# aghasemzadeh/OpenMPL

Measured on AMD Instinct MI355X. Metric: poses/sec (V=4, J=17, batch=1024 per GPU) fp32, higher is better.
Workload: dtype f32; 1 GPU; Human3.6M config: V=4 J=17 batch=1024 fp32, CHOSEN flag set, depth 12, DIM 32, heads 8; global_batch=1024, parallelism=single GPU

## Files before the change

openmpl_amd/csrc/h2_phase.hpp:

```cpp
#pragma once
#include <mutex>
#include <type_traits>

#include "gemm_common.hpp"

namespace mpl {

typedef _Float16 f16x8 __attribute__((ext_vector_type(8)));
typedef __bf16 bf16x8 __attribute__((ext_vector_type(8)));
typedef unsigned u32x4 __attribute__((ext_vector_type(4)));
typedef unsigned u32x2 __attribute__((ext_vector_type(2)));

constexpr int H2_RG = 2 * 1024;
constexpr int H2_A = 4 * H2_RG;
constexpr int H2_W = 18 * 1024;
constexpr int H2_STAGE = H2_A + H2_W;
constexpr int H2_NST = 6;
constexpr int H2_VEC = H2_NST * H2_STAGE;
constexpr int H2_LDS_BYTES = H2_VEC + 4096;
constexpr int H2_DW_RES = 80 * 1024;
constexpr int H2_FAIL = H2_VEC + 4092;
constexpr int H2_T0 = 5;
constexpr int H2_MAX_WGS = 1024;
constexpr int H2_ATT_TS = 3 * BN + 4;
// ... 173 lines not shown
        const float4 a = pv4(row, 32 * p + 4 * kq), b = pv4(row, 32 * p + 16 + 4 * kq);
        float4 sa = {1.f, 1.f, 1.f, 1.f}, sb = {1.f, 1.f, 1.f, 1.f};
        if (NP == 2) { sa = ld4(so + 32 * p + 4 * kq); sb = ld4(so + 32 * p + 16 + 4 * kq); }
        const float x[8] = {a.x * sa.x, a.y * sa.y, a.z * sa.z, a.w * sa.w, b.x * sb.x, b.y * sb.y, b.z * sb.z, b.w * sb.w};
        h2_emit_frag<NP>(WT, cbase, 4 * g_out + p, (unsigned)(rg * strip + (kq * 16 + li) * 16), x);
    }
    for (int t = tid; t < BM * 2; t += 512) {
        const int li = t & 15, kq = (t >> 4) & 1, rg = t >> 5;
        if (rg < rg_lo || rg >= rg_lo + rgs) continue;
        const int row = rg * 16 + li;
        const float4 a = pv4(row, 128 + 4 * kq);
        float4 sa = {1.f, 1.f, 1.f, 1.f};
        if (NP == 2) sa = ld4(so + 128 + 4 * kq);
        const float x[8] = {a.x * sa.x, a.y * sa.y, a.z * sa.z, a.w * sa.w, 0.f, 0.f, 0.f, 0.f};
        h2_emit_tail<NP>(WT, cbase, 4 * Go + (g_out >> 2), (unsigned)(rg * strip + ((g_out & 3) * 16 + li) * 16 + kq * 8), x,
                         ((Dq / BK) & 1) && (g_out >> 2) == (Go >> 2) - 1);
    }
}

__device__ __forceinline__ bool h2_att_in_registers(int ntok, int hd, int rpt) {
    return (ntok == 2 || ntok == 4 || ntok == 8) && (hd == 68 || hd == BN) && rpt == BM;
}

template <int EPI, bool LNF, int NPASS, int NTW, bool CHAIN, int WC, int RT = 1, int NP = 2, bool ACT = true, bool DW = false>
__device__ __forceinline__ bool h2_phase(const H2Args& a, char* smem, int tid, int wave, int slot0, int tm, int tn,
                                         unsigned* chain, unsigned chain_need, bool arrive = true, int rg_lo = 0, int rgs = 4) {
    static_assert(ACT || (RT == 1 && CHAIN), "loader-only waves exist in the row-narrow stack only");
    static_assert(!DW || (RT == 1 && CHAIN && NP == 2), "direct-W form: 16-row teams of the fp16x2 stack");
    constexpr int ABYTES = RT * 4 * H2_RG;
    constexpr int STAGE = ABYTES + H2_W;
    constexpr int NST = RT == 1 ? H2_NST : 4;
    constexpr int APW = 2 * RT;
    static_assert(NST * STAGE <= H2_VEC, "ring too large");
    static_assert(RT == 1 || (RT == 2 && CHAIN && NP == 2 && EPI != H2_EPI_ATT && NPASS <= 2), "two row tiles per stage: proj / fc1 / fc2 of the fp16x2 stack");
    constexpr bool RAWX = LNF && NP == 2;
    constexpr bool P2 = RT == 1;
    constexpr int DIST = P2 ? NST - 1 : NST;
    constexpr bool LEAD = NTW == H2_T0;
    constexpr bool HAS_A = LEAD && ACT;
    const bool WT = CHAIN && !a.plain;
    const int lane = tid & 63;
    const int rg = DW ? rg_lo : (wave & 3);
    const int li = lane & 15, kq = lane >> 4;
    const int M = a.M, N = a.N, K = a.K;
    const int m0 = tm * RT * a.rpt, n0 = NPASS == 2 ? tn * (2 * BN) : tn * BN;
    const int Dq = N / 3;
    const int KT = h2_ksteps(K, NP), G = K / BN;
    const int T = NPASS * KT;
    auto colbase = [&](int pass) -> int { return NPASS == 3 ? pass * Dq + n0 : n0 + pass * BN; };
    const unsigned long long t_entry = (H2_DBG && a.dbg) ? __builtin_amdgcn_s_memtime() : 0;

    const int row_l = rg * 16 + li;
    bool row_ok[RT];
    int row[RT];
#pragma unroll
    for (int rt = 0; rt < RT; ++rt) {
        row_ok[rt] = row_l < a.rpt && m0 + rt * a.rpt + row_l < M;
        row[rt] = row_ok[rt] ? m0 + rt * a.rpt + row_l : (M - 1);
    }

    const int w_first = RT == 1 ? (LEAD ? 10 + 2 * wave : (wave < 6 ? 3 * (wave - 4) : 6 + 2 * (wave - 6)))
                                : (LEAD ? 14 + wave : (wave < 6 ? 4 * (wave - 4) : 8 + 3 * (wave - 6)));
    static_assert(RT == 1 ? (LEAD ? WC == H2_WC0 : (WC == H2_WC1 || WC == H2_WC2))
                          : (LEAD ? WC == H2_R2_WC0 : (WC == H2_R2_WC1 || WC == H2_R2_WC2)), "W pieces per wave");
    constexpr int w_cnt = WC;
    unsigned voW = (unsigned)(lane * 16 + w_first * 1024);
    unsigned voA[RT], voT[RT];
#pragma unroll
    for (int rt = 0; rt < RT; ++rt) {
        voA[rt] = (unsigned)(lane * 16);
        voT[rt] = 0;
        if (RAWX) {
            voA[rt] = (unsigned)(((size_t)(row[rt] - m0) * a.ldx + 4 * kq) * 4);
            voT[rt] = (unsigned)(((size_t)(row[rt] - m0) * a.ldx + 136 * kq + 128) * 4);
        }
        asm volatile("" : "+v"(voA[rt]), "+v"(voT[rt]));
    }
    asm volatile("" : "+v"(voW));
    const unsigned lds0 = (unsigned)(uintptr_t)(__attribute__((address_space(3))) char*)smem;
    int iw_t = 0, iw_g = 0, ia_t = 0, ia_kt = 0;
    unsigned iw_slot = 0, ia_slot = 0;
    const char* is_w[NPASS];
#pragma unroll
    for (int g = 0; g < NPASS; ++g) is_w[g] = a.W2 + (size_t)(colbase(g) / BN) * KT * H2_W;
    const char* is_a[RT];
#pragma unroll
    for (int rt = 0; rt < RT; ++rt)
        is_a[rt] = RAWX ? reinterpret_cast<const char*>(a.X + (size_t)m0 * a.ldx)
                       : a.A2 + (((size_t)tm * RT + rt) * 4 + (wave & 3)) * KT * H2_RG;
    int hotc[NPASS];
#pragma unroll
    for (int g = 0; g < NPASS; ++g) {
        hotc[g] = 0;
        if (H2_ABL & 64) is_w[g] = a.W2 + (size_t)tn * 17 * H2_W;
    }
    auto adv_w = [&](int g) {
        is_w[g] += H2_W;
        if (H2_ABL & 64) {
            if (++hotc[g] == (NP == 2 ? 16 : 8)) {
                hotc[g] = 0;
                is_w[g] -= (NP == 2 ? 16 : 8) * H2_W;
            }
        }
    };
// ... 22 lines not shown
                    asm volatile("s_mov_b32 m0, %2\n\ts_nop 0\n\tglobal_load_lds_dwordx4 %0, %1\n\tglobal_load_lds_dwordx4 %0, %1 offset:1024"
                                 : : "v"(voA[rt]), "s"(is_a[rt]), "s"(dst) : "memory");
                is_a[rt] += H2_RG;
            } else {
                const bool full = ia_kt < 4 * G;
                const char* src = full ? is_a[rt] + (size_t)(136 * (ia_kt >> 2) + 32 * (ia_kt & 3)) * 4 : is_a[rt] + (size_t)(136 * 4 * (ia_kt - 4 * G)) * 4;
                const char* src2 = src + (full ? 64 : 16);
                const unsigned vo = full ? voA[rt] : voT[rt];
                if (CHAIN)
                    asm volatile("s_mov_b32 m0, %3\n\ts_nop 0\n\tglobal_load_lds_dwordx4 %0, %1 sc1\n\ts_mov_b32 m0, %4\n\ts_nop 0\n\tglobal_load_lds_dwordx4 %0, %2 sc1"
                                 : : "v"(vo), "s"(src), "s"(src2), "s"(dst), "s"(dst + 1024u) : "memory");
                else
                    asm volatile("s_mov_b32 m0, %3\n\ts_nop 0\n\tglobal_load_lds_dwordx4 %0, %1\n\ts_mov_b32 m0, %4\n\ts_nop 0\n\tglobal_load_lds_dwordx4 %0, %2"
                                 : : "v"(vo), "s"(src), "s"(src2), "s"(dst), "s"(dst + 1024u) : "memory");
            }
        }
        ++ia_kt;
    };
    auto issue_w = [&]() {
        const unsigned keep = dma_m0_save();
#pragma unroll
        for (int g = 0; g < NPASS; ++g)
            if (g == iw_g) {
                w_pieces(is_w[g], lds0 + iw_slot + (unsigned)(ABYTES + w_first * 1024));
                adv_w(g);
            }
        if (++iw_g == NPASS) iw_g = 0;
        dma_m0_restore(keep);
        ++iw_t;
        iw_slot += STAGE;
        if (iw_slot == NST * STAGE) iw_slot = 0;
    };
    auto issue_a = [&]() {
        if ((ia_t % NPASS) == 0 && HAS_A) {
            const unsigned keep = dma_m0_save();
            a_pieces(ia_slot);
            dma_m0_restore(keep);
        }
        ++ia_t;
        ia_slot += STAGE;
        if (ia_slot == NST * STAGE) ia_slot = 0;
    };
    auto refill_fast = [&](auto wp_c, auto ai_c, unsigned slot) {
        constexpr int g = decltype(wp_c)::value;
        constexpr bool with_a = decltype(ai_c)::value;
        const unsigned keep = dma_m0_save();
        w_pieces(is_w[g], lds0 + slot + (unsigned)(ABYTES + w_first * 1024));
// ... 53 lines not shown
        dw_fetch(std::integral_constant<int, 1>{}, 1 / NPASS);
        dw_fetch(std::integral_constant<int, 2>{}, 2 / NPASS);
        if constexpr (PD == 4) dw_fetch(std::integral_constant<int, 3>{}, 3 / NPASS);
    } else {
        issue_w();
    }
    if (CHAIN) {
        if (!LEAD && wave == 7 && !arrived) {
            const unsigned lim = 1u << a.spin_log2;
            unsigned spin = 0;
            for (; spin < lim; ++spin) {
                if (__hip_atomic_load(chain, __ATOMIC_RELAXED, __HIP_MEMORY_SCOPE_AGENT) >= chain_need) break;
                __builtin_amdgcn_s_sleep(2);
            }
            if (spin == lim && lane == 0) {
                *reinterpret_cast<volatile unsigned*>(smem + H2_FAIL) = 1u;
                if (a.err_ws) __hip_atomic_store(a.err_ws, 1u, __ATOMIC_RELAXED, __HIP_MEMORY_SCOPE_AGENT);
                if (a.err_host) __hip_atomic_store(a.err_host, 1u, __ATOMIC_RELAXED, __HIP_MEMORY_SCOPE_SYSTEM);
                asm volatile("s_waitcnt vmcnt(0) lgkmcnt(0)" ::: "memory");
            }
        }
        __builtin_amdgcn_s_barrier();
        asm volatile("" ::: "memory");
        if (*reinterpret_cast<volatile unsigned*>(smem + H2_FAIL)) {
            asm volatile("s_waitcnt vmcnt(0)" ::: "memory");
            return false;
        }
    }
    const unsigned long long t_chain = (H2_DBG == 2 && a.dbg) ? __builtin_amdgcn_s_memtime() : 0;
    if constexpr (!DW) {
        issue_a();
    } else {
        const int rows_lo = m0 + rg_lo * 16 + li;
        const int rowa = (rg_lo * 16 + li < a.rpt && rows_lo < M) ? rows_lo : (M - 1);
        const unsigned vA = RAWX ? (unsigned)(((size_t)(rowa - m0) * a.ldx + 4 * kq) * 4) : (unsigned)(lane * 16);
        const unsigned vT = RAWX ? (unsigned)(((size_t)(rowa - m0) * a.ldx + 136 * kq + 128) * 4) : 0u;
        const char* abase = RAWX ? reinterpret_cast<const char*>(a.X + (size_t)m0 * a.ldx) : a.A2 + ((size_t)tm * 4 + rg_lo) * KT * H2_RG;
        const unsigned keep = dma_m0_save();
        for (int i = wave; i < 2 * KT; i += 8) {
            const int kt = i >> 1, half = i & 1;
            const char* src;
            unsigned vo;
            if (RAWX) {
                const bool full = kt < 4 * G;
                src = full ? abase + (size_t)(136 * (kt >> 2) + 32 * (kt & 3)) * 4 + half * 64 : abase + (size_t)(136 * 4 * (kt - 4 * G)) * 4 + half * 16;
                vo = full ? vA : vT;
            } else {
                src = abase + (size_t)i * 1024;
                vo = vA;
            }
            asm volatile("s_mov_b32 m0, %2\n\ts_nop 0\n\tglobal_load_lds_dwordx4 %0, %1 sc1" : : "v"(vo), "s"(src), "s"(lds0 + (unsigned)i * 1024u) : "memory");
        }
        dma_m0_restore(keep);
    }
    constexpr unsigned ST_LDS = DW ? 72u * 1024u  : (RT == 2 ? NST * STAGE : STAGE);
    constexpr bool ST_DMA = NPASS >= 2 || RT == 2;
    static_assert(RT == 1 || ST_LDS + 16384 <= H2_VEC, "statistics rows overlap the epilogue vectors");
    float4 st_raw[4];
    if (LNF) {
        const int ns = K / BN;
        if constexpr (ST_DMA) {
            const int hpr = ns >> 1;
            if (lane < 16 * hpr) {
                const unsigned inv = 65536u / (unsigned)hpr + 1u;
                const int lq = (int)(((unsigned)lane * inv) >> 16);
#pragma unroll
                for (int rt = 0; rt < RT; ++rt) {
                    int r = m0 + rt * a.rpt + 16 * rg + lq;
                    r = r < M ? r : M - 1;
                    const float* g = a.stats + ((size_t)r * ns + 2 * (lane - lq * hpr)) * 2;
                    unsigned keep;
                    if (CHAIN)
                        asm volatile("s_mov_b32 %0, m0\n\ts_mov_b32 m0, %2\n\ts_nop 0\n\tglobal_load_lds_dwordx4 %1, off sc1\n\ts_mov_b32 m0, %0"
                                     : "=&s"(keep) : "v"(g), "s"(lds0 + ST_LDS + (unsigned)(wave * 1024 + rt * 8192)) : "memory");
                    else
                        asm volatile("s_mov_b32 %0, m0\n\ts_mov_b32 m0, %2\n\ts_nop 0\n\tglobal_load_lds_dwordx4 %1, off\n\ts_mov_b32 m0, %0"
                                     : "=&s"(keep) : "v"(g), "s"(lds0 + ST_LDS + (unsigned)(wave * 1024 + rt * 8192)) : "memory");
                }
            }
        } else {

            const float* sp = a.stats + (size_t)row[0] * ns * 2;
#pragma unroll
            for (int i = 0; i < 4; ++i) st_raw[i] = (2 * i < ns) ? ld4(sp + 4 * i) : float4{0.f, 0.f, 0.f, 0.f};
        }
    }
    if constexpr (!DW) {
#pragma unroll
        for (int t = 1; t < DIST; ++t) {
            issue_w();
            issue_a();
        }
    }
    const float ainv = (!LNF && a.a_inv) ? a.a_inv[0] : 1.0f;

    float4 rv[RT][NTW];
    auto epilogue_operands = [&]() {
        if constexpr (EPI == H2_EPI_RES && DW) {
#pragma unroll
            for (int n = 0; n < NTW; ++n)
// ... 60 lines not shown
        const f16x8* bs = reinterpret_cast<const f16x8*>(smem + slot + ABYTES) + slot0 * 2 * 64 + lane;
#pragma unroll
        for (int n = 0; n < NTW; ++n) {
            f[n][0] = bs[(n * 2 + 0) * 64];
            f[n][1] = bs[(n * 2 + 1) * 64];
        }
    };
    auto slot_after = [&](unsigned sl) -> unsigned { return sl + STAGE == NST * STAGE ? 0u : sl + STAGE; };
    auto mfma_row = [&](f32x4 (&accp)[RT][NTW], const f16x8 (&af)[RT][2], int ap, const f16x8 (&bf)[NTW][2], int bp) {
#pragma unroll
        for (int rt = 0; rt < RT; ++rt)
#pragma unroll
            for (int n = 0; n < NTW; ++n)
                if (!(H2_ABL & 8)) {
                    if constexpr (NP == 2)
                        accp[rt][n] = __builtin_amdgcn_mfma_f32_16x16x32_f16(bf[n][bp], af[rt][ap], accp[rt][n], 0, 0, 0);
                    else
                        accp[rt][n] = __builtin_amdgcn_mfma_f32_16x16x32_bf16(__builtin_bit_cast(bf16x8, bf[n][bp]), __builtin_bit_cast(bf16x8, af[rt][ap]),
                                                                              accp[rt][n], 0, 0, 0);
                }
    };
    unsigned long long t_land = 0;
    {
        if constexpr (DW) {
            asm volatile("s_waitcnt vmcnt(0)" ::: "memory");
        } else if (HAS_A) {
            constexpr int LATER = P2 ? 2 * WC + APW * (NPASS == 1 ? 2 : 1) : (DIST - 1) * WC + APW * ((DIST - 1) / NPASS);
            static_assert(LATER < 64, "vmcnt is 6 bits");
            asm volatile("s_waitcnt vmcnt(%0)" ::"n"(LATER) : "memory");
        } else {
            asm volatile("s_waitcnt vmcnt(%0)" ::"n"(P2 ? 2 * WC : (DIST - 1) * WC) : "memory");
        }
        if (H2_DBG == 2 && a.dbg) t_land = __builtin_amdgcn_s_memtime();
        {
            if (LNF) {
                const int ns = K / BN;
#pragma unroll
                for (int rt = 0; rt < RT; ++rt) {
                    if constexpr (ST_DMA) {
                        const float* sl = reinterpret_cast<const float*>(smem + ST_LDS + wave * 1024 + rt * 8192) + li * ns * 2;
#pragma unroll
                        for (int i = 0; i < 4; ++i) st_raw[i] = (2 * i < ns) ? ld4(sl + 4 * i) : float4{0.f, 0.f, 0.f, 0.f};
                    }
                    float st[16];
#pragma unroll
                    for (int i = 0; i < 4; ++i) {
                        st[4 * i] = st_raw[i].x; st[4 * i + 1] = st_raw[i].y; st[4 * i + 2] = st_raw[i].z; st[4 * i + 3] = st_raw[i].w;
                    }
                    float msum = 0.f;
#pragma unroll
                    for (int i = 0; i < 8; ++i) msum += (i < ns) ? st[2 * i] : 0.f;
                    const float mean = msum / (float)ns;
                    float m2 = 0.f;
#pragma unroll
                    for (int i = 0; i < 8; ++i) {
                        const float d = st[2 * i] - mean;
                        m2 += (i < ns) ? fmaf((float)BN * d, d, st[2 * i + 1]) : 0.f;
                    }
                    const float rs = 1.0f / sqrtf(fmaf(m2, 1.0f / (float)K, a.eps));
                    if constexpr (NP == 2) {
                        cv_a[rt] = row_ok[rt] ? rs * H2_SA : 0.f;
                        cv_b[rt] = row_ok[rt] ? -mean * (rs * H2_SA) : 0.f;
                    } else {
                        cv_a[rt] = rs;
                        cv_b[rt] = mean;
                    }
                }
                asm volatile("s_waitcnt lgkmcnt(0)" ::: "memory");
            }
        }
        __builtin_amdgcn_s_barrier();
        asm volatile("" ::: "memory");
        if constexpr (ACT && !DW) {
            read_a(0, A0);
            if (RAWX) finish_a(A0);
            read_b(0, B0);
        }
        if constexpr (DW && RAWX) {
            for (int kt = wave; kt < KT; kt += 8) {
                char* p = smem + kt * 2048 + lane * 16;
                cvr0[0] = *reinterpret_cast<const float4*>(p);
                cvr1[0] = *reinterpret_cast<const float4*>(p + 1024);
                finish_a(A0);
                *reinterpret_cast<f16x8*>(p) = A0[0][0];
                *reinterpret_cast<f16x8*>(p + 1024) = A0[0][1];
            }
            asm volatile("s_waitcnt lgkmcnt(0)" ::: "memory");
            __builtin_amdgcn_s_barrier();
            asm volatile("" ::: "memory");
        }
    }
    const unsigned long long t_loop = (H2_DBG && a.dbg) ? __builtin_amdgcn_s_memtime() : 0;
    unsigned long long t_vm = 0, t_bar = 0, t_mm = 0;
    unsigned slot_c = 0;
    auto stage = [&](auto rem_c, auto wp_c, f32x4 (&accp)[RT][NTW], const f16x8 (&a_cur)[RT][2], f16x8 (&a_nxt)[RT][2],
                     const f16x8 (&b_cur)[NTW][2], f16x8 (&b_nxt)[NTW][2], auto nha_c, auto sync_c) {
        constexpr int REM = decltype(rem_c)::value;
        constexpr bool FAST = REM == 0;
        constexpr bool SYNC = !(P2 && FAST) || decltype(sync_c)::value;
        constexpr bool next_has_a = decltype(nha_c)::value;
        constexpr bool more = FAST || REM > 1;
        constexpr bool RF = FAST || REM > DIST;
        constexpr int g0 = decltype(wp_c)::value;
        asm volatile("" : "+s"(slot_c));
        const unsigned slot_n = slot_after(slot_c);
        const unsigned slot_p = slot_c == 0 ? (unsigned)((NST - 1) * STAGE) : slot_c - STAGE;
        unsigned long long w0 = 0, w1 = 0;
        if (H2_DBG && a.dbg) w0 = __builtin_amdgcn_s_memtime();
        if (more && SYNC) {
            if (FAST) {
                if (P2) {
                    constexpr int na = ((g0 + 3) % NPASS == 0 ? 1 : 0) + ((g0 + 4) % NPASS == 0 ? 1 : 0);
                    if (HAS_A) asm volatile("s_waitcnt vmcnt(%0)" ::"n"(2 * WC + APW * na) : "memory");
                    else asm volatile("s_waitcnt vmcnt(%0)" ::"n"(2 * WC) : "memory");
                } else {
                    constexpr int na = ((g0 + 2) % NPASS == 0 ? 1 : 0) + ((g0 + 3) % NPASS == 0 ? 1 : 0) +
                                       (NST > 4 ? ((g0 + 4) % NPASS == 0 ? 1 : 0) + ((g0 + 5) % NPASS == 0 ? 1 : 0) : 0);
                    static_assert(NST == 4 || NST == 6, "in-flight stages of the one-barrier-per-stage form");
                    static_assert((NST - 2) * WC + APW * na < 64, "vmcnt is 6 bits");
                    if (HAS_A) asm volatile("s_waitcnt vmcnt(%0)" ::"n"((NST - 2) * WC + APW * na) : "memory");
                    else asm volatile("s_waitcnt vmcnt(%0)" ::"n"((NST - 2) * WC) : "memory");
                }
            } else {
                constexpr int ahead = (REM - 1 < DIST - 1 ? REM - 1 : DIST - 1) - 1;
                constexpr int per = HAS_A ? WC + (NPASS == 1 ? APW : 0) : WC;
                constexpr int allow = ahead > 0 ? ahead * per : 0;
                static_assert(allow < 64, "vmcnt is 6 bits");
                asm volatile("s_waitcnt vmcnt(%0)" ::"n"(allow) : "memory");
            }
            if (H2_DBG && a.dbg) { w1 = __builtin_amdgcn_s_memtime(); t_vm += w1 - w0; }
            asm volatile("s_waitcnt lgkmcnt(0)" ::: "memory");
            if (!(H2_ABL & 32)) __builtin_amdgcn_s_barrier();
            asm volatile("" ::: "memory");
            if (H2_DBG && a.dbg) t_bar += __builtin_amdgcn_s_memtime() - w1;
        }
        const f16x8* bs = reinterpret_cast<const f16x8*>(smem + slot_n + ABYTES) + slot0 * 2 * 64 + lane;
        auto rd_b = [&](int n) {
            if (more && n < NTW && !(H2_ABL & 1)) {
                b_nxt[n][0] = bs[(n * 2 + 0) * 64];
                b_nxt[n][1] = bs[(n * 2 + 1) * 64];
            }
        };
        auto loads = [&]() {
            if constexpr (ACT) {
                if (more && next_has_a && !(H2_ABL & 4)) read_a(slot_n, a_nxt);
                rd_b(0); rd_b(1); rd_b(2); rd_b(3); rd_b(4);
            }
            constexpr int gr = (g0 + DIST) % NPASS;
            if (RF && !(H2_ABL & 2))
                refill_fast(std::integral_constant<int, gr>{}, std::integral_constant<bool, gr == 0>{}, P2 ? slot_p : slot_c);
            if (REM == 4 && ACT) epilogue_operands();
        };
        __builtin_amdgcn_sched_barrier(0);
        if (!LEAD) {
            loads();
            __builtin_amdgcn_sched_barrier(0);
        }
        unsigned long long m0 = 0;
        if (H2_DBG && a.dbg) m0 = __builtin_amdgcn_s_memtime();
        if constexpr (!ACT) {
        } else if constexpr (NP == 2) {
            mfma_row(accp, a_cur, 1, b_cur, 0);
            mfma_row(accp, a_cur, 0, b_cur, 1);
            mfma_row(accp, a_cur, 0, b_cur, 0);
        } else {
            mfma_row(accp, a_cur, 0, b_cur, 0);
            mfma_row(accp, a_cur, 1, b_cur, 1);
        }
        __builtin_amdgcn_sched_barrier(0);
        if (H2_DBG && a.dbg) t_mm += __builtin_amdgcn_s_memtime() - m0;
        if (LEAD) loads();
        if (RAWX && ACT && more && next_has_a && !(H2_ABL & 16)) finish_a(a_nxt);
        __builtin_amdgcn_sched_barrier(0);
// ... 102 lines not shown
            if constexpr (PD == 4 && (PD + 3) % NPASS == 0) {
                if (rest == PD + 3) {
                    do tail(tail, std::integral_constant<int, PD + 3>{}, Z{}); while (--tail_rep);
                }
            }
            epilogue_operands();
        }
    } else {
    int t = 0;
    for (; t + U - 1 + NST < T; t += U) {
        step(R0{}, std::integral_constant<int, 0>{});
        step(R0{}, std::integral_constant<int, 1 % U>{});
        if constexpr (NPASS >= 2) {
            step(R0{}, std::integral_constant<int, 2 % U>{});
            step(R0{}, std::integral_constant<int, 3 % U>{});
        }
        if constexpr (NPASS == 3) {
            step(R0{}, std::integral_constant<int, 4 % U>{});
            step(R0{}, std::integral_constant<int, 5 % U>{});
        }
    }
    constexpr int TAIL_A = (NST + U - 1) / U * U;
    constexpr int TAIL_B = (NST - NPASS + U - 1) / U * U + NPASS;
    if (T - t == TAIL_A) tail(tail, std::integral_constant<int, TAIL_A>{}, std::integral_constant<int, 0>{});
    else tail(tail, std::integral_constant<int, TAIL_B>{}, std::integral_constant<int, 0>{});
    }

    const unsigned long long t_epi = (H2_DBG && a.dbg) ? __builtin_amdgcn_s_memtime() : 0;
    auto tile_of = [&](int n) -> int { return h2_slot_tile(slot0 + n); };
    auto value4 = [&](int p, int rt, int n, float (&v)[4]) {
        const int cl = 16 * tile_of(n) + 4 * kq;
        const bool ok = cl + 3 < BN;
        const float* vecs = reinterpret_cast<const float*>(smem + H2_VEC) + p * 2 * BN + (ok ? cl : 0);
        const float4 cv = ld4(vecs), sv = ld4(vecs + BN);
        const float c4[4] = {cv.x, cv.y, cv.z, cv.w};
        const float s4[4] = {sv.x, sv.y, sv.z, sv.w};
#pragma unroll
        for (int r = 0; r < 4; ++r) {
            float t;
            if constexpr (NP == 2) t = fmaf(acc[p][rt][n][r], LNF ? s4[r] : s4[r] * ainv, c4[r]);
            else if constexpr (LNF) t = fmaf(cv_a[rt], fmaf(-cv_b[rt], s4[r], acc[p][rt][n][r]), c4[r]);
            else t = acc[p][rt][n][r] + c4[r];
            if (EPI == H2_EPI_GELU) t = gelu_as(t);
            v[r] = ok ? t : 0.f;
        }
    };
// ... 65 lines not shown
            for (int n = 0; n < NTW; ++n) {
                const bool h1 = two_heads && 4 * tile_of(n) + kq >= 17;
                float km[4] = {0.f, 0.f, 0.f, 0.f};
                if constexpr (NTK > 4) {
#pragma unroll
                    for (int c = 0; c < 4; ++c) km[c] = mirror(kv[n][c]);
                }
#pragma unroll
                for (int r = 0; r < NTK; ++r) {
                    float d = qv[n][0] * xpart(kv[n][0], km[0], r);
                    d = fmaf(qv[n][1], xpart(kv[n][1], km[1], r), d);
                    d = fmaf(qv[n][2], xpart(kv[n][2], km[2], r), d);
                    d = fmaf(qv[n][3], xpart(kv[n][3], km[3], r), d);
                    s0[r] += h1 ? 0.f : d;
                    s1[r] += h1 ? d : 0.f;
                }
            }
#pragma unroll
            for (int r = 0; r < NTK; ++r) {
                s0[r] = xor16_add(s0[r]); s0[r] = xor32_add(s0[r]);
                s1[r] = xor16_add(s1[r]); s1[r] = xor32_add(s1[r]);
            }
            float* xs = reinterpret_cast<float*>(smem) + rt * (2 * BM * 2 * NTK);
            const int half = slot0 ? 1 : 0;
            __syncthreads();
            if (kq == 0) {
#pragma unroll
                for (int r = 0; r < NTK; ++r) {
                    xs[(half * BM + row_l) * 2 * NTK + r] = s0[r];
                    xs[(half * BM + row_l) * 2 * NTK + NTK + r] = s1[r];
                }
            }
            __syncthreads();
            float p0[NTK], p1[NTK];
            {
                const float scale = 1.0f / sqrtf((float)a.att_hd);
                float t0[NTK], t1[NTK];
#pragma unroll
                for (int r = 0; r < NTK; ++r) {
                    t0[r] = (xs[row_l * 2 * NTK + r] + xs[(BM + row_l) * 2 * NTK + r]) * scale;
                    t1[r] = (xs[row_l * 2 * NTK + NTK + r] + xs[(BM + row_l) * 2 * NTK + NTK + r]) * scale;
                }
                auto softmax = [](const float (&t)[NTK], float (&pr)[NTK]) {
                    float mx = t[0];
#pragma unroll
                    for (int r = 1; r < NTK; ++r) mx = fmaxf(mx, t[r]);
// ... 38 lines not shown
                return __builtin_bit_cast(float, r);
            };
            const bool two_heads = a.att_hd == 68;
            float s0[4] = {0.f, 0.f, 0.f, 0.f}, s1[4] = {0.f, 0.f, 0.f, 0.f};
    #pragma unroll
            for (int n = 0; n < NTW; ++n) {
                const bool h1 = two_heads && 4 * tile_of(n) + kq >= 17;
    #pragma unroll
                for (int j = 0; j < 4; ++j) {
                    float d = qv[n][0] * quad(kv[n][0], j);
                    d = fmaf(qv[n][1], quad(kv[n][1], j), d);
                    d = fmaf(qv[n][2], quad(kv[n][2], j), d);
                    d = fmaf(qv[n][3], quad(kv[n][3], j), d);
                    s0[j] += h1 ? 0.f : d;
                    s1[j] += h1 ? d : 0.f;
                }
            }
    #pragma unroll
            for (int j = 0; j < 4; ++j) {
                s0[j] = xor16_add(s0[j]); s0[j] = xor32_add(s0[j]);
                s1[j] = xor16_add(s1[j]); s1[j] = xor32_add(s1[j]);
            }
            float* xs = reinterpret_cast<float*>(smem) + rt * (2 * BM * 8);
            const int half = slot0 ? 1 : 0;
            __syncthreads();
            if (kq == 0) {
                st4(xs + (half * BM + row_l) * 8, float4{s0[0], s0[1], s0[2], s0[3]});
                st4(xs + (half * BM + row_l) * 8 + 4, float4{s1[0], s1[1], s1[2], s1[3]});
            }
            __syncthreads();
            float p0[4], p1[4];
            {
                const float4 a0 = ld4(xs + row_l * 8), a1 = ld4(xs + row_l * 8 + 4);
                const float4 b0 = ld4(xs + (BM + row_l) * 8), b1 = ld4(xs + (BM + row_l) * 8 + 4);
                const float scale = 1.0f / sqrtf((float)a.att_hd);
                const float t0[4] = {(a0.x + b0.x) * scale, (a0.y + b0.y) * scale, (a0.z + b0.z) * scale, (a0.w + b0.w) * scale};
                const float t1[4] = {(a1.x + b1.x) * scale, (a1.y + b1.y) * scale, (a1.z + b1.z) * scale, (a1.w + b1.w) * scale};
                auto softmax4 = [](const float (&t)[4], float (&pr)[4]) {
                    const float mx = fmaxf(fmaxf(t[0], t[1]), fmaxf(t[2], t[3]));
                    const float e0 = __expf(t[0] - mx), e1 = __expf(t[1] - mx), e2 = __expf(t[2] - mx), e3 = __expf(t[3] - mx);
                    const float inv = 1.0f / ((e0 + e1) + (e2 + e3));
                    pr[0] = e0 * inv; pr[1] = e1 * inv; pr[2] = e2 * inv; pr[3] = e3 * inv;
                };
                softmax4(t0, p0);
                softmax4(t1, p1);
            }
// ... 88 lines not shown
                            for (int r = 0; r < 4; ++r) vals[rt][n][r] *= so4[r];
                        }
                    }
#pragma unroll
                    for (int q = 0; q < 2; ++q) {
                        const float x[8] = {vals[rt][2 * q][0], vals[rt][2 * q][1], vals[rt][2 * q][2], vals[rt][2 * q][3],
                                            vals[rt][2 * q + 1][0], vals[rt][2 * q + 1][1], vals[rt][2 * q + 1][2], vals[rt][2 * q + 1][3]};
                        h2_emit_frag<NP>(WT, cbase, 4 * g_out + (slot0 ? 2 : 0) + q, (unsigned)(lane * 16), x);
                    }
                    if (NTW == H2_T0 && kq < 2) {
                        const float x[8] = {vals[rt][NTW - 1][0], vals[rt][NTW - 1][1], vals[rt][NTW - 1][2], vals[rt][NTW - 1][3], 0.f, 0.f, 0.f, 0.f};
                        h2_emit_tail<NP>(WT, cbase, 4 * Go + (g_out >> 2), (unsigned)(((g_out & 3) * 16 + li) * 16 + kq * 8), x,
                                         ((N / BK) & 1) && (g_out >> 2) == (Go >> 2) - 1);
                    }
                  }
                }
            }
        }
        if (H2_DBG && a.dbg) t_st = __builtin_amdgcn_s_memtime();
        if constexpr (EPI == H2_EPI_RES) {
            if (a.stats_out) {
                constexpr int XR = RT * 64;
                float* xch = reinterpret_cast<float*>(smem);
                const int half = slot0 ? 1 : 0;
                float sum[RT];
#pragma unroll
                for (int rt = 0; rt < RT; ++rt) {
                    sum[rt] = 0.f;
#pragma unroll
                    for (int n = 0; n < NTW; ++n) sum[rt] += (vals[rt][n][0] + vals[rt][n][1]) + (vals[rt][n][2] + vals[rt][n][3]);
                    sum[rt] = xor16_add(sum[rt]);
                    sum[rt] = xor32_add(sum[rt]);
                }
                __syncthreads();
#pragma unroll
                for (int rt = 0; rt < RT; ++rt)
                    if (kq == 0) xch[half * XR + rt * 64 + row_l] = sum[rt];
                __syncthreads();
                float mean[RT];
#pragma unroll
                for (int rt = 0; rt < RT; ++rt) {
                    mean[rt] = (xch[rt * 64 + row_l] + xch[XR + rt * 64 + row_l]) * (1.0f / (float)BN);
                    float q = 0.f;
#pragma unroll
                    for (int n = 0; n < NTW; ++n) {
                        const bool ok = 16 * tile_of(n) + 4 * kq + 3 < BN;
// ... 13 lines not shown
                    if (half == 0 && kq == 0 && row_ok[rt]) {
                        const u32x2 h = {__builtin_bit_cast(unsigned, mean[rt]),
                                         __builtin_bit_cast(unsigned, xch[2 * XR + rt * 64 + row_l] + xch[3 * XR + rt * 64 + row_l])};
                        h2_st8(WT, a.stats_out + (size_t)m0 * Go * 2, (unsigned)(((row[rt] - m0) * Go + n0 / BN) * 8), h);
                    }
            }
        }
    }
    }
    if (CHAIN) {
        asm volatile("s_waitcnt vmcnt(0)" ::: "memory");
        __syncthreads();
        if (tid == 0 && arrive) __hip_atomic_fetch_add(chain, 1u, __ATOMIC_RELAXED, __HIP_MEMORY_SCOPE_AGENT);
    }
    if (H2_DBG && a.dbg) {
        if (!t_st) t_st = __builtin_amdgcn_s_memtime();
        asm volatile("s_waitcnt vmcnt(0)" ::: "memory");
        const unsigned long long t_end = __builtin_amdgcn_s_memtime();
        if (lane == 0) {
            unsigned long long* o = a.dbg + (size_t)(blockIdx.x * 8 + wave) * 8;
            o[0] = t_entry; o[1] = t_loop; o[2] = t_epi; o[3] = t_st; o[4] = t_end; o[5] = t_vm; o[6] = t_bar; o[7] = t_mm;
            if (H2_DBG == 2) { o[5] = t_chain; o[6] = t_land; }
        }
    }
    return true;
}

template <int EPI, bool LNF, int NPASS, int NP = 2>
__global__ __launch_bounds__(512, 2) void h2_gemm_kernel(const H2Args a) {
    extern __shared__ __attribute__((aligned(1024))) char smem[];
    const int tid = threadIdx.x;
    const int wave = __builtin_amdgcn_readfirstlane(tid >> 6);
    int tm, tn;
    {
        const int b = blockIdx.x;
        if ((a.grid_m & 7) == 0) {
            const int per = a.grid_m >> 3;
            const int xcd = b & 7, i = b >> 3;
            tm = xcd * per + (i % per);
            tn = i / per;
        } else {
            tm = b % a.grid_m;
            tn = b / a.grid_m;
        }
    }
    if (wave < 4) h2_phase<EPI, LNF, NPASS, H2_T0, false, H2_WC0, 1, NP>(a, smem, tid, wave, 0, tm, tn, nullptr, 0u);
// ... 39 lines not shown
                  s.spin_log2, plain};
}
template <int NP>
__device__ __forceinline__ H2Args h2_args_res(const H2StackArgs& s, const char* w, bool fc2, int D, int G, int plain) {
    if (H2_ABL & 64) w = s.w[0][0];
    const int K = fc2 ? 2 * D : D;
    const float* v = h2_trailer<NP>(w, D, K);
    return H2Args{fc2 ? s.hid2 : s.att2, nullptr, 0, w, v, v + D, nullptr, nullptr, nullptr, s.x, D, s.x, D, NP == 1 ? s.x16 : nullptr,
                  s.stats, s.M, D, K, s.rpt, s.n_tiles, G, s.eps, 0, 0, s.dbg, s.err_ws, s.err_host, s.spin_log2, plain};
}

__device__ __forceinline__ void h2_publish_xcd(const H2StackArgs& s, int team, int tid) {
    if (tid == 0) {
        unsigned xcc;
        asm volatile("s_getreg_b32 %0, hwreg(HW_REG_XCC_ID)" : "=s"(xcc));
        __hip_atomic_fetch_or(s.xcc + team, 1u << (xcc & 15u), __ATOMIC_RELAXED, __HIP_MEMORY_SCOPE_AGENT);
    }
}
__device__ __forceinline__ int h2_team_on_one_xcd(const H2StackArgs& s, int team) {
    const unsigned m = __hip_atomic_load(s.xcc + team, __ATOMIC_RELAXED, __HIP_MEMORY_SCOPE_AGENT);
    return (s.plain_ok && m != 0u && (m & (m - 1u)) == 0u) ? 1 : 0;
}

template <int NP>
__global__ __launch_bounds__(512, 2) void h2_stack_kernel(const H2StackArgs s) {
    extern __shared__ __attribute__((aligned(1024))) char smem[];
    const int tid = threadIdx.x;
    const int wave_s = __builtin_amdgcn_readfirstlane(tid >> 6);
    const int G = s.G, D = s.D;
    int team, tn;
    {
        const int b = blockIdx.x;
        team = (b & 7) + 8 * ((b >> 3) / G);
        tn = (b >> 3) % G;
        if (team >= s.n_teams) return;
    }
    if (tid == 0) *reinterpret_cast<volatile unsigned*>(smem + H2_FAIL) = 0u;
    h2_publish_xcd(s, team, tid);
    int plain = 0, seen = 0;
    __syncthreads();
    for (int tile0 = team; tile0 < s.n_tiles; tile0 += s.n_teams) {
        unsigned need = 0;
        for (int ph = 0; ph < s.n_phases; ++ph, need += G) {
            if (!seen && ph >= 2) {
                plain = __builtin_amdgcn_readfirstlane(h2_team_on_one_xcd(s, team));
                seen = 1;
            }
            int wvp = wave_s, tile = tile0, tnp = tn;
            asm volatile("" : "+s"(wvp), "+s"(tile), "+s"(tnp));
            int tidp = wvp * 64 + (int)__builtin_amdgcn_mbcnt_hi(~0u, __builtin_amdgcn_mbcnt_lo(~0u, 0u));
            asm volatile("" : "+v"(tidp));
            const int wv = wvp;
            unsigned* ctr = s.counters + tile;
            const char* const* w = s.w[ph >> 2];
            bool ok = true;
            if (s.inject > 0 && ph == s.inject && tile == 0 && tnp == 0) return;
            switch (ph & 3) {
                case 0: {
                    H2Args a = h2_args_qkv<NP>(s, w[0], D, G, plain);
                    if (wv < 4) ok = h2_phase<H2_EPI_ATT, true, 3, H2_T0, true, H2_WC0, 1, NP>(a, smem, tidp, wv, 0, tile, tnp, ctr, need);
                    else if (wv < 6) ok = h2_phase<H2_EPI_ATT, true, 3, NT - H2_T0, true, H2_WC1, 1, NP>(a, smem, tidp, wv, H2_T0, tile, tnp, ctr, need);
                    else ok = h2_phase<H2_EPI_ATT, true, 3, NT - H2_T0, true, H2_WC2, 1, NP>(a, smem, tidp, wv, H2_T0, tile, tnp, ctr, need);
                    break;
                }
                case 2: {
                    H2Args a = h2_args_fc1<NP>(s, w[2], D, G, plain);
                    if (wv < 4) ok = h2_phase<H2_EPI_GELU, true, 2, H2_T0, true, H2_WC0, 1, NP>(a, smem, tidp, wv, 0, tile, tnp, ctr, need);
                    else if (wv < 6) ok = h2_phase<H2_EPI_GELU, true, 2, NT - H2_T0, true, H2_WC1, 1, NP>(a, smem, tidp, wv, H2_T0, tile, tnp, ctr, need);
                    else ok = h2_phase<H2_EPI_GELU, true, 2, NT - H2_T0, true, H2_WC2, 1, NP>(a, smem, tidp, wv, H2_T0, tile, tnp, ctr, need);
                    break;
                }
                default: {
                    const bool fc2 = (ph & 3) == 3;
                    H2Args a = h2_args_res<NP>(s, fc2 ? w[3] : w[1], fc2, D, G, plain);
                    if (wv < 4) ok = h2_phase<H2_EPI_RES, false, 1, H2_T0, true, H2_WC0, 1, NP>(a, smem, tidp, wv, 0, tile, tnp, ctr, need);
                    else if (wv < 6) ok = h2_phase<H2_EPI_RES, false, 1, NT - H2_T0, true, H2_WC1, 1, NP>(a, smem, tidp, wv, H2_T0, tile, tnp, ctr, need);
                    else ok = h2_phase<H2_EPI_RES, false, 1, NT - H2_T0, true, H2_WC2, 1, NP>(a, smem, tidp, wv, H2_T0, tile, tnp, ctr, need);
                    break;
                }
            }
            if (!ok) return;
        }
    }
}

template <int NP>
__global__ __launch_bounds__(512, 2) void h2_stack2_kernel(const H2StackArgs s) {
    static_assert(NP == 2, "the two-tile stage exists in the fp16x2 engine only");
    extern __shared__ __attribute__((aligned(1024))) char smem[];
    const int tid = threadIdx.x;
    const int wave_s = __builtin_amdgcn_readfirstlane(tid >> 6);
    const int G = s.G, D = s.D;
    int team, tn;
    {
        const int b = blockIdx.x;
        team = (b & 7) + 8 * ((b >> 3) / G);
        tn = (b >> 3) % G;
        if (team >= s.n_teams) return;
    }
    if (tid == 0) *reinterpret_cast<volatile unsigned*>(smem + H2_FAIL) = 0u;
// ... 324 lines not shown
```

Baseline: 816,200 poses/s.

## Prefetch next phase's weight tiles into the LDS ring during the current phase tail

Adds a cross-phase weight prefetch to the persistent stack kernel. During the last DIST stages of each GEMM phase, freed ring slots are filled with the next phase's W pieces, and the next phase starts from the ring position left behind and skips reissuing those loads. The aim is to hide the weight-load latency at the start of each phase behind the previous phase's tail and epilogue. The cost is more intricate vmcnt accounting, relocated statistics and exchange buffers, and a risk of LDS overlap between in-flight prefetch and epilogue scratch.

```diff
diff --git a/openmpl_amd/csrc/h2_phase.hpp b/openmpl_amd/csrc/h2_phase.hpp
--- a/openmpl_amd/csrc/h2_phase.hpp
+++ b/openmpl_amd/csrc/h2_phase.hpp
@@ -219,11 +219,22 @@
     return (ntok == 2 || ntok == 4 || ntok == 8) && (hd == 68 || hd == BN) && rpt == BM;
 }
 
-template <int EPI, bool LNF, int NPASS, int NTW, bool CHAIN, int WC, int RT = 1, int NP = 2, bool ACT = true, bool DW = false>
+struct H2Pf {
+    unsigned base;
+    int pre;
+    const char* nw;
+    unsigned pstride;
+    int npass;
+};
+constexpr int H2_PF_MIN_T = 12;
+
+template <int EPI, bool LNF, int NPASS, int NTW, bool CHAIN, int WC, int RT = 1, int NP = 2, bool ACT = true, bool DW = false, bool PF = false>
 __device__ __forceinline__ bool h2_phase(const H2Args& a, char* smem, int tid, int wave, int slot0, int tm, int tn,
-                                         unsigned* chain, unsigned chain_need, bool arrive = true, int rg_lo = 0, int rgs = 4) {
+                                         unsigned* chain, unsigned chain_need, bool arrive = true, int rg_lo = 0, int rgs = 4,
+                                         H2Pf* pf = nullptr) {
     static_assert(ACT || (RT == 1 && CHAIN), "loader-only waves exist in the row-narrow stack only");
     static_assert(!DW || (RT == 1 && CHAIN && NP == 2), "direct-W form: 16-row teams of the fp16x2 stack");
+    static_assert(!PF || (RT == 1 && CHAIN && ACT && !DW), "cross-phase W prefetch: the whole-tile chain form only");
     constexpr int ABYTES = RT * 4 * H2_RG;
     constexpr int STAGE = ABYTES + H2_W;
     constexpr int NST = RT == 1 ? H2_NST : 4;
@@ -245,6 +256,20 @@
     const int KT = h2_ksteps(K, NP), G = K / BN;
     const int T = NPASS * KT;
     auto colbase = [&](int pass) -> int { return NPASS == 3 ? pass * Dq + n0 : n0 + pass * BN; };
+    unsigned ring0 = 0;
+    bool pre = false, pf_on = false;
+    const char* pf_nw = nullptr;
+    unsigned pf_ps = 0;
+    int pf_np = 1;
+    if constexpr (PF) {
+        ring0 = pf->base;
+        pre = pf->pre != 0;
+        pf_nw = pf->nw;
+        pf_ps = pf->pstride;
+        pf_np = pf->npass;
+        pf_on = pf_nw != nullptr && !(H2_ABL & 64);
+        if (EPI == H2_EPI_ATT && !h2_att_in_registers(a.att_ntok, a.att_hd, a.rpt)) pf_on = false;
+    }
     const unsigned long long t_entry = (H2_DBG && a.dbg) ? __builtin_amdgcn_s_memtime() : 0;
 
     const int row_l = rg * 16 + li;
@@ -276,7 +301,7 @@
     asm volatile("" : "+v"(voW));
     const unsigned lds0 = (unsigned)(uintptr_t)(__attribute__((address_space(3))) char*)smem;
     int iw_t = 0, iw_g = 0, ia_t = 0, ia_kt = 0;
-    unsigned iw_slot = 0, ia_slot = 0;
+    unsigned iw_slot = ring0, ia_slot = ring0;
     const char* is_w[NPASS];
 #pragma unroll
     for (int g = 0; g < NPASS; ++g) is_w[g] = a.W2 + (size_t)(colbase(g) / BN) * KT * H2_W;
@@ -345,7 +370,7 @@
 #pragma unroll
         for (int g = 0; g < NPASS; ++g)
             if (g == iw_g) {
-                w_pieces(is_w[g], lds0 + iw_slot + (unsigned)(ABYTES + w_first * 1024));
+                if (!pre) w_pieces(is_w[g], lds0 + iw_slot + (unsigned)(ABYTES + w_first * 1024));
                 adv_w(g);
             }
         if (++iw_g == NPASS) iw_g = 0;
@@ -445,7 +470,9 @@
         }
         __builtin_amdgcn_s_barrier();
         asm volatile("" ::: "memory");
-        if (*reinterpret_cast<volatile unsigned*>(smem + H2_FAIL)) {
+        unsigned lost = *reinterpret_cast<volatile unsigned*>(smem + H2_FAIL);
+        if constexpr (PF) lost = (unsigned)__builtin_amdgcn_readfirstlane((int)lost);
+        if (lost) {
             asm volatile("s_waitcnt vmcnt(0)" ::: "memory");
             return false;
         }
@@ -479,6 +506,7 @@
     constexpr unsigned ST_LDS = DW ? 72u * 1024u  : (RT == 2 ? NST * STAGE : STAGE);
     constexpr bool ST_DMA = NPASS >= 2 || RT == 2;
     static_assert(RT == 1 || ST_LDS + 16384 <= H2_VEC, "statistics rows overlap the epilogue vectors");
+    const unsigned st_lds = PF ? (ring0 + STAGE == NST * STAGE ? 0u : ring0 + (unsigned)STAGE) : ST_LDS;
     float4 st_raw[4];
     if (LNF) {
         const int ns = K / BN;
@@ -495,10 +523,10 @@
                     unsigned keep;
                     if (CHAIN)
                         asm volatile("s_mov_b32 %0, m0\n\ts_mov_b32 m0, %2\n\ts_nop 0\n\tglobal_load_lds_dwordx4 %1, off sc1\n\ts_mov_b32 m0, %0"
-                                     : "=&s"(keep) : "v"(g), "s"(lds0 + ST_LDS + (unsigned)(wave * 1024 + rt * 8192)) : "memory");
+                                     : "=&s"(keep) : "v"(g), "s"(lds0 + st_lds + (unsigned)(wave * 1024 + rt * 8192)) : "memory");
                     else
                         asm volatile("s_mov_b32 %0, m0\n\ts_mov_b32 m0, %2\n\ts_nop 0\n\tglobal_load_lds_dwordx4 %1, off\n\ts_mov_b32 m0, %0"
-                                     : "=&s"(keep) : "v"(g), "s"(lds0 + ST_LDS + (unsigned)(wave * 1024 + rt * 8192)) : "memory");
+                                     : "=&s"(keep) : "v"(g), "s"(lds0 + st_lds + (unsigned)(wave * 1024 + rt * 8192)) : "memory");
                 }
             }
         } else {
@@ -605,7 +633,10 @@
     };
     unsigned long long t_land = 0;
     {
-        if constexpr (DW) {
+        if (PF && pre) {
+            if constexpr (HAS_A) asm volatile("s_waitcnt vmcnt(%0)" ::"n"(APW * (NPASS == 1 ? 2 : 1)) : "memory");
+            else asm volatile("s_waitcnt vmcnt(0)" ::: "memory");
+        } else if constexpr (DW) {
             asm volatile("s_waitcnt vmcnt(0)" ::: "memory");
         } else if (HAS_A) {
             constexpr int LATER = P2 ? 2 * WC + APW * (NPASS == 1 ? 2 : 1) : (DIST - 1) * WC + APW * ((DIST - 1) / NPASS);
@@ -621,7 +652,7 @@
 #pragma unroll
                 for (int rt = 0; rt < RT; ++rt) {
                     if constexpr (ST_DMA) {
-                        const float* sl = reinterpret_cast<const float*>(smem + ST_LDS + wave * 1024 + rt * 8192) + li * ns * 2;
+                        const float* sl = reinterpret_cast<const float*>(smem + st_lds + wave * 1024 + rt * 8192) + li * ns * 2;
 #pragma unroll
                         for (int i = 0; i < 4; ++i) st_raw[i] = (2 * i < ns) ? ld4(sl + 4 * i) : float4{0.f, 0.f, 0.f, 0.f};
                     }
@@ -655,9 +686,9 @@
         __builtin_amdgcn_s_barrier();
         asm volatile("" ::: "memory");
         if constexpr (ACT && !DW) {
-            read_a(0, A0);
+            read_a(ring0, A0);
             if (RAWX) finish_a(A0);
-            read_b(0, B0);
+            read_b(ring0, B0);
         }
         if constexpr (DW && RAWX) {
             for (int kt = wave; kt < KT; kt += 8) {
@@ -675,7 +706,7 @@
     }
     const unsigned long long t_loop = (H2_DBG && a.dbg) ? __builtin_amdgcn_s_memtime() : 0;
     unsigned long long t_vm = 0, t_bar = 0, t_mm = 0;
-    unsigned slot_c = 0;
+    unsigned slot_c = ring0;
     auto stage = [&](auto rem_c, auto wp_c, f32x4 (&accp)[RT][NTW], const f16x8 (&a_cur)[RT][2], f16x8 (&a_nxt)[RT][2],
                      const f16x8 (&b_cur)[NTW][2], f16x8 (&b_nxt)[NTW][2], auto nha_c, auto sync_c) {
         constexpr int REM = decltype(rem_c)::value;
@@ -709,7 +740,10 @@
                 constexpr int per = HAS_A ? WC + (NPASS == 1 ? APW : 0) : WC;
                 constexpr int allow = ahead > 0 ? ahead * per : 0;
                 static_assert(allow < 64, "vmcnt is 6 bits");
-                asm volatile("s_waitcnt vmcnt(%0)" ::"n"(allow) : "memory");
+                constexpr int allow_pf = allow + (PF && REM <= DIST ? (DIST - REM) * WC : 0);
+                static_assert(allow_pf < 64, "vmcnt is 6 bits");
+                if (PF && REM < DIST && pf_on) asm volatile("s_waitcnt vmcnt(%0)" ::"n"(allow_pf) : "memory");
+                else asm volatile("s_waitcnt vmcnt(%0)" ::"n"(allow) : "memory");
             }
             if (H2_DBG && a.dbg) { w1 = __builtin_amdgcn_s_memtime(); t_vm += w1 - w0; }
             asm volatile("s_waitcnt lgkmcnt(0)" ::: "memory");
@@ -732,6 +766,16 @@
             constexpr int gr = (g0 + DIST) % NPASS;
             if (RF && !(H2_ABL & 2))
                 refill_fast(std::integral_constant<int, gr>{}, std::integral_constant<bool, gr == 0>{}, P2 ? slot_p : slot_c);
+            if constexpr (PF && !FAST && REM <= DIST) {
+                if (pf_on) {
+                    constexpr int j = DIST - REM;
+                    const unsigned g = pf_np == 1 ? 0u : (pf_np == 2 ? (unsigned)(j & 1) : (unsigned)(j % 3));
+                    const unsigned kt = pf_np == 1 ? (unsigned)j : (pf_np == 2 ? (unsigned)(j >> 1) : (unsigned)(j / 3));
+                    const unsigned keep = dma_m0_save();
+                    w_pieces(pf_nw + (size_t)g * pf_ps + (size_t)kt * H2_W, lds0 + slot_p + (unsigned)(ABYTES + w_first * 1024));
+                    dma_m0_restore(keep);
+                }
+            }
             if (REM == 4 && ACT) epilogue_operands();
         };
         __builtin_amdgcn_sched_barrier(0);
@@ -880,6 +924,8 @@
     }
     constexpr int TAIL_A = (NST + U - 1) / U * U;
     constexpr int TAIL_B = (NST - NPASS + U - 1) / U * U + NPASS;
+    static_assert(!PF || (TAIL_A > TAIL_B ? TAIL_A : TAIL_B) + DIST - 2 <= H2_PF_MIN_T,
+                  "H2_PF_MIN_T admits a prefetched phase whose tail would under-wait");
     if (T - t == TAIL_A) tail(tail, std::integral_constant<int, TAIL_A>{}, std::integral_constant<int, 0>{});
     else tail(tail, std::integral_constant<int, TAIL_B>{}, std::integral_constant<int, 0>{});
     }
@@ -991,6 +1037,7 @@
                 s1[r] = xor16_add(s1[r]); s1[r] = xor32_add(s1[r]);
             }
             float* xs = reinterpret_cast<float*>(smem) + rt * (2 * BM * 2 * NTK);
+            static_assert(!PF || RT * 2 * BM * 2 * NTK * (int)sizeof(float) <= ABYTES, "exchange buffer beyond the A region of slot 0");
             const int half = slot0 ? 1 : 0;
             __syncthreads();
             if (kq == 0) {
@@ -1075,6 +1122,7 @@
                 s1[j] = xor16_add(s1[j]); s1[j] = xor32_add(s1[j]);
             }
             float* xs = reinterpret_cast<float*>(smem) + rt * (2 * BM * 8);
+            static_assert(!PF || RT * 2 * BM * 8 * (int)sizeof(float) <= ABYTES, "exchange buffer beyond the A region of slot 0 (PF: W prefetch in flight)");
             const int half = slot0 ? 1 : 0;
             __syncthreads();
             if (kq == 0) {
@@ -1209,6 +1257,7 @@
             if (a.stats_out) {
                 constexpr int XR = RT * 64;
                 float* xch = reinterpret_cast<float*>(smem);
+                static_assert(!PF || 4 * XR * (int)sizeof(float) <= ABYTES, "exchange buffer beyond the A region of slot 0");
                 const int half = slot0 ? 1 : 0;
                 float sum[RT];
 #pragma unroll
@@ -1268,6 +1317,10 @@
             o[0] = t_entry; o[1] = t_loop; o[2] = t_epi; o[3] = t_st; o[4] = t_end; o[5] = t_vm; o[6] = t_bar; o[7] = t_mm;
             if (H2_DBG == 2) { o[5] = t_chain; o[6] = t_land; }
         }
+    }
+    if constexpr (PF) {
+        pf->base = pf_on ? slot_c : 0u;
+        pf->pre = pf_on ? 1 : 0;
     }
     return true;
 }
@@ -1353,6 +1406,13 @@
     return (s.plain_ok && m != 0u && (m & (m - 1u)) == 0u) ? 1 : 0;
 }
 
+template <int EPI, bool LNF, int NPASS, int NTW, int WC, int NP>
+__device__ __forceinline__ bool h2_phase_pf(const H2Args& a, char* smem, int tid, int wave, int slot0, int tm, int tn,
+                                            unsigned* chain, unsigned chain_need, H2Pf& pf) {
+    return h2_phase<EPI, LNF, NPASS, NTW, true, WC, 1, NP, true, false, true>(a, smem, tid, wave, slot0, tm, tn, chain, chain_need,
+                                                                              true, 0, 4, &pf);
+}
+
 template <int NP>
 __global__ __launch_bounds__(512, 2) void h2_stack_kernel(const H2StackArgs s) {
     extern __shared__ __attribute__((aligned(1024))) char smem[];
@@ -1370,6 +1430,7 @@
     h2_publish_xcd(s, team, tid);
     int plain = 0, seen = 0;
     __syncthreads();
+    H2Pf pf{0u, 0, nullptr, 0u, 1};
     for (int tile0 = team; tile0 < s.n_tiles; tile0 += s.n_teams) {
         unsigned need = 0;
         for (int ph = 0; ph < s.n_phases; ++ph, need += G) {
@@ -1386,27 +1447,42 @@
             const char* const* w = s.w[ph >> 2];
             bool ok = true;
             if (s.inject > 0 && ph == s.inject && tile == 0 && tnp == 0) return;
+            {
+                int nph = ph + 1;
+                if (nph == s.n_phases) nph = tile0 + s.n_teams < s.n_tiles ? 0 : -1;
+                pf.nw = nullptr;
+                if (nph >= 0) {
+                    const int kind = nph & 3;
+                    const int npass = kind == 0 ? 3 : (kind == 2 ? 2 : 1);
+                    const int ktn = h2_ksteps(kind == 3 ? 2 * D : D, NP);
+                    if (npass * ktn >= H2_PF_MIN_T) {
+                        pf.nw = s.w[nph >> 2][kind] + (size_t)(npass == 3 ? tnp : npass * tnp) * ktn * H2_W;
+                        pf.pstride = (unsigned)((npass == 3 ? G : 1) * ktn * H2_W);
+                        pf.npass = npass;
+                    }
+                }
+            }
             switch (ph & 3) {
                 case 0: {
                     H2Args a = h2_args_qkv<NP>(s, w[0], D, G, plain);
-                    if (wv < 4) ok = h2_phase<H2_EPI_ATT, true, 3, H2_T0, true, H2_WC0, 1, NP>(a, smem, tidp, wv, 0, tile, tnp, ctr, need);
-                    else if (wv < 6) ok = h2_phase<H2_EPI_ATT, true, 3, NT - H2_T0, true, H2_WC1, 1, NP>(a, smem, tidp, wv, H2_T0, tile, tnp, ctr, need);
-                    else ok = h2_phase<H2_EPI_ATT, true, 3, NT - H2_T0, true, H2_WC2, 1, NP>(a, smem, tidp, wv, H2_T0, tile, tnp, ctr, need);
+                    if (wv < 4) ok = h2_phase_pf<H2_EPI_ATT, true, 3, H2_T0, H2_WC0, NP>(a, smem, tidp, wv, 0, tile, tnp, ctr, need, pf);
+                    else if (wv < 6) ok = h2_phase_pf<H2_EPI_ATT, true, 3, NT - H2_T0, H2_WC1, NP>(a, smem, tidp, wv, H2_T0, tile, tnp, ctr, need, pf);
+                    else ok = h2_phase_pf<H2_EPI_ATT, true, 3, NT - H2_T0, H2_WC2, NP>(a, smem, tidp, wv, H2_T0, tile, tnp, ctr, need, pf);
                     break;
                 }
                 case 2: {
                     H2Args a = h2_args_fc1<NP>(s, w[2], D, G, plain);
-                    if (wv < 4) ok = h2_phase<H2_EPI_GELU, true, 2, H2_T0, true, H2_WC0, 1, NP>(a, smem, tidp, wv, 0, tile, tnp, ctr, need);
-                    else if (wv < 6) ok = h2_phase<H2_EPI_GELU, true, 2, NT - H2_T0, true, H2_WC1, 1, NP>(a, smem, tidp, wv, H2_T0, tile, tnp, ctr, need);
-                    else ok = h2_phase<H2_EPI_GELU, true, 2, NT - H2_T0, true, H2_WC2, 1, NP>(a, smem, tidp, wv, H2_T0, tile, tnp, ctr, need);
+                    if (wv < 4) ok = h2_phase_pf<H2_EPI_GELU, true, 2, H2_T0, H2_WC0, NP>(a, smem, tidp, wv, 0, tile, tnp, ctr, need, pf);
+                    else if (wv < 6) ok = h2_phase_pf<H2_EPI_GELU, true, 2, NT - H2_T0, H2_WC1, NP>(a, smem, tidp, wv, H2_T0, tile, tnp, ctr, need, pf);
+                    else ok = h2_phase_pf<H2_EPI_GELU, true, 2, NT - H2_T0, H2_WC2, NP>(a, smem, tidp, wv, H2_T0, tile, tnp, ctr, need, pf);
                     break;
                 }
                 default: {
                     const bool fc2 = (ph & 3) == 3;
                     H2Args a = h2_args_res<NP>(s, fc2 ? w[3] : w[1], fc2, D, G, plain);
-                    if (wv < 4) ok = h2_phase<H2_EPI_RES, false, 1, H2_T0, true, H2_WC0, 1, NP>(a, smem, tidp, wv, 0, tile, tnp, ctr, need);
-                    else if (wv < 6) ok = h2_phase<H2_EPI_RES, false, 1, NT - H2_T0, true, H2_WC1, 1, NP>(a, smem, tidp, wv, H2_T0, tile, tnp, ctr, need);
-                    else ok = h2_phase<H2_EPI_RES, false, 1, NT - H2_T0, true, H2_WC2, 1, NP>(a, smem, tidp, wv, H2_T0, tile, tnp, ctr, need);
+                    if (wv < 4) ok = h2_phase_pf<H2_EPI_RES, false, 1, H2_T0, H2_WC0, NP>(a, smem, tidp, wv, 0, tile, tnp, ctr, need, pf);
+                    else if (wv < 6) ok = h2_phase_pf<H2_EPI_RES, false, 1, NT - H2_T0, H2_WC1, NP>(a, smem, tidp, wv, H2_T0, tile, tnp, ctr, need, pf);
+                    else ok = h2_phase_pf<H2_EPI_RES, false, 1, NT - H2_T0, H2_WC2, NP>(a, smem, tidp, wv, H2_T0, tile, tnp, ctr, need, pf);
                     break;
                 }
             }
```

Result: faster. 845,400 poses/s (median of 6 runs) (+3.6%).
